# mlelarge/graph_neural_net

Measured on AMD Instinct MI355X. Metric: graph-pairs/sec FGNN fwd+bwd, N=50 regular pairs, higher is better.
Workload: dtype f32

## Files before the change

graph_neural_net_amd/_lib.py:

```python
import ctypes as C
import os

import torch

_HERE = os.path.dirname(os.path.abspath(__file__))
LIB_PATH = os.environ.get('FGNN_LIB') or os.path.join(_HERE, 'libfgnn_hip.so')

FGNN_H = 32
FGNN_TILE = 32
FGNN_MAX_DEPTH = 3
FGNN_RANGE_WG = 256
FGNN_LSAP_MAX_N = 2048
FGNN_QAP_MAX_N = 256
FGNN_QAPW_MAX_N = 256
FGNN_SPECTRAL_MAX_N = 256
FGNN_SPECTRAL_MAX_POWERS = 8
FGNN_SCORE_SPLIT = 4

c_float_p = C.c_void_p


class Slab(C.Structure):
    _fields_ = [('ptr', C.c_void_p), ('gstride', C.c_longlong), ('ldp', C.c_longlong), ('C', C.c_int),
                ('nrm', C.c_void_p), ('beta', C.c_void_p)]
# ... 38 lines not shown
                ('dxb', C.c_void_p), ('dxb_gstride', C.c_longlong), ('dxb_ld', C.c_longlong),
                ('accumulate_dx', C.c_int), ('accumulate_dxb', C.c_int),
                ('wpart', C.c_void_p)]


class Mlp64PackJob(C.Structure):
    _fields_ = [('W', C.c_void_p * 3), ('bias', C.c_void_p * 3), ('cin', C.c_int), ('packed', C.c_void_p)]


class MlpBwdArgs(C.Structure):
    _fields_ = [('G', C.c_int), ('N', C.c_int), ('depth', C.c_int),
                ('nvalid', C.c_void_p),
                ('a', Slab), ('b', Slab),
                ('W', C.c_void_p * FGNN_MAX_DEPTH),
                ('bias', C.c_void_p * FGNN_MAX_DEPTH),
                ('dy', C.c_void_p), ('dgstride', C.c_longlong), ('ldd', C.c_longlong),
                ('z', C.c_void_p), ('zgstride', C.c_longlong), ('ldz', C.c_longlong),
                ('coef', C.c_void_p), ('s12', C.c_void_p), ('znrm', C.c_void_p),
                ('dxa', C.c_void_p), ('dxa_gstride', C.c_longlong), ('dxa_ld', C.c_longlong),
                ('dxb', C.c_void_p), ('dxb_gstride', C.c_longlong), ('dxb_ld', C.c_longlong),
                ('accumulate_a', C.c_int), ('accumulate_b', C.c_int),
                ('wpart', C.c_void_p), ('s12part', C.c_void_p), ('packed', C.c_void_p),
                ('s12tiles', C.c_void_p), ('s12_out', C.c_void_p), ('xbits', C.c_void_p), ('xdeg', C.c_void_p),
                ('ranges', C.c_void_p), ('cu_share', C.c_int)]


class Slab16(C.Structure):
    _fields_ = [('ptr', C.c_void_p), ('gstride', C.c_longlong), ('ldp', C.c_longlong), ('C', C.c_int),
                ('nrm', C.c_void_p), ('beta', C.c_void_p)]


class MlpFwd16Args(C.Structure):
    _fields_ = [('G', C.c_int), ('N', C.c_int), ('ldr', C.c_int), ('depth', C.c_int), ('nmlp', C.c_int),
                ('nvalid', C.c_void_p),
                ('a', Slab16), ('b', Slab16),
                ('z', C.c_void_p * 2), ('ldz', C.c_longlong),
                ('part', C.c_void_p * 2), ('cnt', C.c_void_p), ('packed', C.c_void_p), ('ranges', C.c_void_p)]


class MlpBwd16Args(C.Structure):
    _fields_ = [('G', C.c_int), ('N', C.c_int), ('ldr', C.c_int), ('depth', C.c_int),
                ('nvalid', C.c_void_p),
                ('a', Slab16), ('b', Slab16),
                ('dy', C.c_void_p), ('dgstride', C.c_longlong), ('ldd', C.c_longlong),
                ('z', C.c_void_p), ('zgstride', C.c_longlong), ('ldz', C.c_longlong),
                ('coef', C.c_void_p),
                ('dxa', C.c_void_p), ('dxa_gstride', C.c_longlong), ('dxa_ld', C.c_longlong),
# ... 60 lines not shown
    'fgnn_mlp64_pack_multi': [C.POINTER(Mlp64PackJob), _I, _VP],
    'fgnn_mlp64_fwd': [C.POINTER(Mlp64Args), _VP],
    'fgnn_mlp64_bwd': [C.POINTER(Mlp64Args), _VP],
    'fgnn_conv1x1': [_VP, _LL, _LL, _VP, _VP, _LL, _LL, _VP, _I, _VP, _I, _I, _I, _I, _VP, _LL, _LL, _VP],
    'fgnn_conv1x1_dw_chunks': [_I, _I],
    'fgnn_conv1x1_dw': [_VP, _LL, _LL, _VP, _VP, _LL, _LL, _VP, _I, _I, _I, _I, _VP, _VP],
    'fgnn_chan_matmul_fwd': [C.POINTER(Slab), C.POINTER(Slab), _VP, _I, _I, _VP, _LL, _LL, _VP],
    'fgnn_chan_matmul_fwd_ord': [C.POINTER(Slab), C.POINTER(Slab), _VP, _I, _I, _VP, _LL, _LL, _VP, _I, _VP],
    'fgnn_chan_matmul_fwd_fin_supported': [_I],
    'fgnn_chan_matmul_fwd_fin': [C.POINTER(Slab), C.POINTER(Slab), _VP, _VP, _VP, _VP, _VP, _F, _VP, _I, _I, _VP, _LL, _LL, _VP],
    'fgnn_chan_matmul_fwd_fin_ord': [C.POINTER(Slab), C.POINTER(Slab), _VP, _VP, _VP, _VP, _VP, _F, _VP, _I, _I, _VP, _LL, _LL, _VP, _I, _VP],
    'fgnn_colmax_fwd': [C.POINTER(Slab), _VP, _I, _I, _VP, _VP, _VP],
    'fgnn_colmax_fwd_fin_supported': [_I],
    'fgnn_colmax_fwd_fin': [C.POINTER(Slab), _VP, _VP, _VP, _F, _VP, _I, _I, _VP, _VP, _VP],
    'fgnn_score_ce_fwd': [_VP, _VP, _VP, _I, _I, _I, _VP, _VP, _VP, _VP],
    'fgnn_score_row_blocks': [_I, _I],
    'fgnn_score_ce_fwd_blocks': [_VP, _VP, _VP, _I, _I, _I, _I, _VP, _VP, _VP, _VP],
    'fgnn_score_ce_bwd': [_VP, _VP, _VP, _VP, _VP, _VP, _I, _I, _I, _VP, _VP, _VP],
    'fgnn_inv_node_count': [_VP, _I, _VP, _VP],
    'fgnn_score_bwd': [_VP, _VP, _VP, _VP, _I, _I, _I, _VP, _VP, _VP],
    'fgnn_ce_fwd': [_VP, _VP, _I, _I, _VP, _VP, _VP],
    'fgnn_ce_bwd': [_VP, _VP, _VP, _VP, _I, _I, _VP, _VP],
    'fgnn_colmax_bwd': [_VP, _VP, _VP, _I, _I, _I, _VP, _LL, _LL, C.POINTER(Slab), _VP, _VP],
    'fgnn_gn_bwd_stats': [_VP, _LL, _LL, _VP, _LL, _LL, _VP, _VP, _I, _I, _I, _VP, _VP],
    'fgnn_gn_bwd_coef': [_VP, _VP, _VP, _I, _I, _I, _VP, _VP, _VP, _VP],
    'fgnn_gn_bwd_coef_tiles': [_VP, _VP, _VP, _I, _I, _I, _VP, _VP, _VP],
    'fgnn_grad_finalize': [_VP, _I, _I, _I, _I, _VP],
    'fgnn_gn_bwd_apply': [_VP, _LL, _LL, _VP, _LL, _LL, _VP, _VP, _I, _I, _I, _VP, _LL, _LL, _VP],
    'fgnn_mlp_bwd': [C.POINTER(MlpBwdArgs), _VP],
    'fgnn_mlp_bwd_x3': [C.POINTER(MlpBwdArgs), _VP],
    'fgnn_mlp_bwd_pair': [C.POINTER(MlpBwdArgs), C.POINTER(MlpBwdArgs), _VP],
    'fgnn_mlp_bwd_t16': [C.POINTER(MlpBwdArgs), _VP],
    'fgnn_mlp_bwd_t16_supported': [C.POINTER(MlpBwdArgs)],
    'fgnn_mlp_bwd_pair_t16': [C.POINTER(MlpBwdArgs), C.POINTER(MlpBwdArgs), _VP],
    'fgnn_mlp_bwd_pair_x3': [C.POINTER(MlpBwdArgs), C.POINTER(MlpBwdArgs), _VP],
    'fgnn_block1_struct_supported': [_I, _I, _I],
    'fgnn_block1_struct_table_floats': [_I],
    'fgnn_block1_struct_ws_floats': [_I, _I],
    'fgnn_block1_struct_rows': [_I, _I],
    'fgnn_block1_struct_fwd': [_VP, _VP, _I, _I, _VP, _VP, _VP, _VP, _VP, C.c_float, _VP, _VP, _VP, _LL, _LL, _VP, _VP, _VP, _VP, _VP, _VP, _VP],
    'fgnn_block1_struct_bwd': [_VP, _VP, _I, _I, _VP, _VP, _VP, _VP, _VP, _VP, _VP, _VP, _LL, _LL, _VP, _VP, _VP, _VP, _VP, _VP],
    'fgnn_block1_struct_fwd_pack': [_VP, _VP, _I, _I, _VP, _VP, _VP, _VP, _VP, C.c_float, _VP, _VP, _VP, _LL, _LL, _VP, _VP, _VP, _VP, _VP, _VP, _VP, _I, _VP],
    'fgnn_block1_struct_fwd16_pack': [_VP, _VP, _I, _I, _I, _VP, _VP, _VP, _VP, _VP, C.c_float, _VP, _VP, _VP, _LL, _LL, _VP, _VP, _VP, _VP, _VP, _VP, _VP, _I, _VP],
    'fgnn_block1_struct_fwd16': [_VP, _VP, _I, _I, _I, _VP, _VP, _VP, _VP, _VP, C.c_float, _VP, _VP, _VP, _LL, _LL, _VP, _VP, _VP, _VP, _VP, _VP, _VP],
    'fgnn_block1_struct_bwd16': [_VP, _VP, _I, _I, _I, _VP, _VP, _VP, _VP, _VP, _VP, _VP, _VP, _LL, _LL, _VP, _VP, _VP, _VP, _VP, _VP],
    'fgnn_mlp_bwd_coef_tiles_supported': [_I, _I],
    'fgnn_mlp_param_count': [_I, _I],
    'fgnn_reduce_partials': [_VP, _I, _I, _VP, _VP],
    'fgnn_chan_matmul_bwd': [C.POINTER(Slab), C.POINTER(Slab), _VP, _LL, _LL, _VP, _I, _I, _VP, _VP, _LL, _LL, _VP, _VP, _VP],
    'fgnn_chan_matmul_bwd_ord': [C.POINTER(Slab), C.POINTER(Slab), _VP, _LL, _LL, _VP, _I, _I, _VP, _VP, _LL, _LL, _VP, _VP, _VP, _I, _VP],
    'fgnn_sum_scale': [_VP, _I, _I, _F, _VP, _VP],
    'fgnn_adam_step': [_VP, _VP, _VP, _VP, _I, C.c_double, C.c_double, C.c_double, C.c_double, _I, C.c_double, _VP],
    'fgnn_adam_step_dev': [_VP, _VP, _VP, _VP, _I, _VP, _VP, _VP],
    'fgnn_expand_adjacency': [_VP, _VP, _I, _I, _VP, _VP],
    'fgnn_pack_adjacency': [_VP, _VP, _I, _I, _VP, _VP, _VP],
    'fgnn_pack_adjacency_ld': [_VP, _VP, _I, _I, _I, _VP, _VP, _VP],
# ... 133 lines not shown
```

graph_neural_net_amd/csrc/mlp_bwd_t16.hip:

```cpp
#include "fgnn_t16.h"
#include "fgnn_pack.h"

namespace {

using namespace t16;

constexpr int BWD_WG = 256;
constexpr int NW = 8;

DEVI float4 coef_from_sums(const float4 n, const float2 sv, float nv) {
    const float m = nv * nv;
    float4 k;
    k.x = n.x;
    k.y = n.y;
    k.z = m > 0.f ? -n.y * sv.y * n.w / m : 0.f;
    k.w = m > 0.f ? -n.y * sv.x / m : 0.f;
    return k;
}
DEVI int graph_nv(const rsrc_t &rnv, bool ragged, int g, int N) {
    const int v = __builtin_amdgcn_raw_buffer_load_b32(rnv, g * 4, 0, 0);
    return __builtin_amdgcn_readfirstlane(ragged ? v : N);
}

template <int CB>
struct Layout16 {
    static constexpr int DEPTH = 3;
    static constexpr PkBwd PK = pk_bwd(32, CB, DEPTH);
    static constexpr int OFF_W0A = PK.off_w1a, OFF_W0B = PK.off_w1b, OFF_W1 = PK.off_wh, OFF_WT1 = PK.off_wt, OFF_WT2 = PK.off_wt + 16;
    static constexpr int OFF_WT0A = PK.off_wt0a, OFF_WT0B = PK.off_wt0b;
    static constexpr int BIAS_F = PK.bias_f;
    static constexpr int WEIGHT_F = pk_pad_floats(PK.floats);
    static constexpr int NSLOT = 5;
    static constexpr int CIN = 32 + CB;
    static constexpr int PCOUNT = 32 * CIN + 32 + (DEPTH - 1) * (32 * 32 + 32);
    static constexpr int TILE_OFF = WEIGHT_F;
    static constexpr int REC_OFF = TILE_OFF + NW * NSLOT * TILE_F;
    static constexpr int WGK_OFF = REC_OFF + NW * 256;
    static constexpr int LIVE_OFF = WGK_OFF + FGNN_BWD_COEF_GRAPHS * 128;
    static constexpr int MAIN_F = LIVE_OFF + LIVE_LIST_CAP + NW;
    static constexpr int RED_F = NW * PCOUNT;
    static constexpr int LDS_F = MAIN_F > RED_F ? MAIN_F : RED_F;
};

template <int CB, bool PKD, bool SKIP, bool DXB>
__global__ __launch_bounds__(64 * NW, 2) void mlp_bwd_t16_kernel(const fgnn_mlp_bwd_args A, const int tpg, const int total_tiles) {
    extern __shared__ __attribute__((aligned(16))) float smem[];
    using L = Layout16<CB>;
    constexpr bool NB = CB == 32;
    const int lane = threadIdx.x & 63, wv = __builtin_amdgcn_readfirstlane(threadIdx.x >> 6);
    const int px = lane & 15, q = lane >> 4;
    const int P2 = A.N * A.N, hpg = 2 * tpg;
    const View va = make_view(A.a.ptr, A.a.gstride, A.a.ldp, A.G);
    const View vb = make_view(A.b.ptr, A.b.gstride, A.b.ldp, A.G);
    PackedSrc ps = {};
    if constexpr (PKD) ps = make_packed_src(A.xbits, A.xdeg, A.G, A.N);
    const View vdy = make_view(A.dy, A.dgstride, A.ldd, A.G);
    const View vz = make_view(A.z, A.zgstride, A.ldz, A.G);
    const View vdxa = make_view(A.dxa, A.dxa_gstride, A.dxa_ld, A.G);
    const View vdxb = make_view(A.dxb, A.dxb_gstride, A.dxb_ld, A.G);

    float *wl = smem;
    float *my = smem + L::TILE_OFF + wv * (L::NSLOT * TILE_F);
    float *XA = my, *XB = my + TILE_F, *S0 = my + 2 * TILE_F, *S1 = my + 3 * TILE_F, *S2 = my + 4 * TILE_F;
    const int lane_base = tile_lane_base(px, q);

    f32x4 dW0a[4], dW0b[4], dW1[4], dW2[4];
    float db0[2] = {0.f, 0.f}, db1[2] = {0.f, 0.f}, db2[2] = {0.f, 0.f}, dbx[2] = {0.f, 0.f};
#pragma unroll
    for (int k = 0; k < 4; ++k) dW0a[k] = dW0b[k] = dW1[k] = dW2[k] = zero4();

    const int nwg = gridDim.x;
    const int qq = total_tiles / nwg, rem = total_tiles % nwg;
    int T0 = blockIdx.x * qq + ((int)blockIdx.x < rem ? (int)blockIdx.x : rem);
    int T1 = T0 + qq + ((int)blockIdx.x < rem ? 1 : 0);
    if constexpr (SKIP) {
        T0 = A.ranges[blockIdx.x];
        T1 = A.ranges[blockIdx.x + 1];
    }
    const int H0 = 2 * T0, H1 = 2 * T1;
// ... 75 lines not shown
            }
            rec[lane] = k4;
            if (NB && A.b.nrm) rec[32 + lane] = reinterpret_cast<const float4 *>(A.b.nrm)[(long long)g * A.b.C + lane];
        }
    };
    auto read_records = [&]() {
#pragma unroll
        for (int s = 0; s < 8; ++s) {
            const float4 k4 = rec[chan_s(s) + chan_q(q)];
            kx[s] = k4.x;
            ky[s] = k4.y;
            kz[s] = k4.z;
            kw[s] = k4.w;
            if (NB && A.b.nrm) {
                const float4 n = rec[32 + chan_s(s) + chan_q(q)];
                mean[s] = n.x;
                av[s] = n.y;
            }
        }
    };

    constexpr int NXB = CB == 32 ? 8 : 1;
    float xa[8], xb[NXB], dyr[8], zr[8];
    auto load_x = [&](int h) {
        const bool act = h < H1;
        const int g = __builtin_amdgcn_readfirstlane(act ? h / hpg : 0);
        const int p = (act ? h - g * hpg : 0) * 16 + px;
        const bool inb = act && p < P2;
        load8(xa, va, lane_voff(va, q, p, inb), g * va.gs4);
        if constexpr (CB == 32) {
            load8(xb, vb, lane_voff(vb, q, p, inb), g * vb.gs4);
        } else if constexpr (PKD) {
            int i, jj;
            row_col(p, A.N, rcpN, i, jj);
            const int ob = (inb && q == 0) ? (i * ps.words + (jj >> 5)) * 4 : OOB_OFF;
            const int od = (inb && q == 1 && i == jj) ? i * 4 : OOB_OFF;
            const unsigned w = (unsigned)__builtin_amdgcn_raw_buffer_load_b32(ps.bits, ob, g * ps.N * ps.words * 4, 0);
            const float d = __builtin_bit_cast(float, __builtin_amdgcn_raw_buffer_load_b32(ps.deg, od, g * ps.N * 4, 0));
            xb[0] = q == 0 ? (((w >> (jj & 31)) & 1u) ? 1.f : 0.f) : d;
        } else {
            xb[0] = buf_load(vb, (inb && q < 2) ? q * vb.ld4 + 4 * p : OOB_OFF, g * vb.gs4);
        }
    };
    auto load_dyz = [&](int h) {
        const bool act = h < H1;
        const int g = __builtin_amdgcn_readfirstlane(act ? h / hpg : 0);
        const int p = (act ? h - g * hpg : 0) * 16 + px;
        const bool inb = act && p < P2;
        load8(dyr, vdy, lane_voff(vdy, q, p, inb), g * vdy.gs4);
        load8(zr, vz, lane_voff(vz, q, p, inb), g * vz.gs4);
    };

    int h = next_half(SKIP ? H0 : H0 + wv);
    load_x(h);
    int cached_g = -1, cur_nv = A.N;

    if (from_tiles) {
        const int g1 = T1 > T0 ? (T1 - 1) / tpg : g0 - 1;
        float2 *scr = reinterpret_cast<float2 *>(smem + L::TILE_OFF);
        const int cc = threadIdx.x & 31, sl = threadIdx.x >> 5;
        for (int g = g0; g <= g1; ++g) {
            float p1 = 0.f, p2 = 0.f;
            constexpr int TS = (64 * NW) / 32, U = 8;
            for (int t0 = sl; t0 < tpg; t0 += TS * U) {
                float2 v[U];
#pragma unroll
                for (int k = 0; k < U; ++k) {
                    const int t = t0 + TS * k;
                    v[k] = reinterpret_cast<const float2 *>(A.s12tiles)[((long long)g * tpg + (t < tpg ? t : 0)) * FGNN_H + cc];
                }
#pragma unroll
                for (int k = 0; k < U; ++k) {
// ... 63 lines not shown
            }
            stage8(XA, lane_base, xa);
            if constexpr (CB == 32) {
                stage8(XB, lane_base, yb);
            } else {
                if (q < 2) XB[8 * q * TLD + px] = yb[0];
            }
            f32x4 acc[2];
            load_bias(acc, wl + L::BIAS_F, 0, q);
            gemm32<L::OFF_W0A>(acc, wl, xa, lane);
            if constexpr (CB == 32) gemm32<L::OFF_W0B>(acc, wl, yb, lane);
            else gemm2<L::OFF_W0B>(acc, wl, q < 2 ? yb[0] : 0.f, lane);
            load_x(hn);
#pragma unroll
            for (int s = 0; s < 8; ++s) h1[s] = relu1(acc[s >> 2][s & 3]);
            stage8(S0, lane_base, h1);
            load_bias(acc, wl + L::BIAS_F, 1, q);
            gemm32<L::OFF_W1>(acc, wl, h1, lane);
#pragma unroll
            for (int s = 0; s < 8; ++s) h2[s] = relu1(acc[s >> 2][s & 3]);
            stage8(S1, lane_base, h2);
        }
        float dpre[8];
#pragma unroll
        for (int s = 0; s < 8; ++s) dpre[s] = fmaf(kz[s], zr[s] - kx[s], fmaf(ky[s], dyr[s], kw[s]));
        if (!full) {
#pragma unroll
            for (int s = 0; s < 8; ++s) dpre[s] = valid ? dpre[s] : 0.f;
        }
        stage8(S2, lane_base, dpre);
        load_dyz(hn);
        __builtin_amdgcn_sched_barrier(0);
        {
            f32x4 a2[2];
            a2[0] = a2[1] = zero4();
            gemm32<L::OFF_WT2>(a2, wl, dpre, lane);
            wgrad16(dW2, db2, S2, S1, lane);
#pragma unroll
            for (int s = 0; s < 8; ++s) dpre[s] = h2[s] > 0.f ? a2[s >> 2][s & 3] : 0.f;
        }
        __builtin_amdgcn_sched_barrier(0);
        stage8(S1, lane_base, dpre);
        {
            f32x4 a2[2];
            a2[0] = a2[1] = zero4();
            gemm32<L::OFF_WT1>(a2, wl, dpre, lane);
// ... 76 lines not shown
            red[32 * CIN + 32 + 1024 + c1] = db1[1];
            red[32 * CIN + 32 + 1056 + 1024 + c0] = db2[0];
            red[32 * CIN + 32 + 1056 + 1024 + c1] = db2[1];
        }
    }
    __syncthreads();
    static_assert(PCOUNT % 4 == 0, "partials are summed four at a time");
    float4 *out = reinterpret_cast<float4 *>(A.wpart + (long long)blockIdx.x * PCOUNT);
    const float4 *part4 = reinterpret_cast<const float4 *>(smem);
    for (int e = threadIdx.x; e < PCOUNT / 4; e += 64 * NW) {
        float4 a = part4[e];
#pragma unroll
        for (int w = 1; w < NW; ++w) {
            const float4 b = part4[w * (PCOUNT / 4) + e];
            a.x += b.x;
            a.y += b.y;
            a.z += b.z;
            a.w += b.w;
        }
        out[e] = a;
    }
}

template <int CB, bool PKD, bool SKIP, bool DXB>
int launch16(const fgnn_mlp_bwd_args *a, int tpg, int total, hipStream_t st) {
    constexpr int LDS = Layout16<CB>::LDS_F * 4;
    static_assert(LDS <= 160 * 1024, "LDS budget");
    static LdsAttrCache attr_cache;
    (void)fgnn_raise_lds(attr_cache, (const void *)mlp_bwd_t16_kernel<CB, PKD, SKIP, DXB>, LDS);
    hipLaunchKernelGGL((mlp_bwd_t16_kernel<CB, PKD, SKIP, DXB>), dim3(a->cu_share == 2 && !SKIP ? BWD_WG / 2 : BWD_WG), dim3(64 * NW), LDS, st, *a,
                       tpg, total);
    FGNN_LAUNCH_CHECK();
    return 0;
}
template <int CB, bool PKD, bool DXB>
int launch16s(const fgnn_mlp_bwd_args *a, int tpg, int total, hipStream_t st) {
    return a->ranges ? launch16<CB, PKD, true, DXB>(a, tpg, total, st) : launch16<CB, PKD, false, DXB>(a, tpg, total, st);
}

}

extern "C" int fgnn_mlp_bwd_t16_supported(const fgnn_mlp_bwd_args *a) {
    if (!a || a->depth != 3 || a->a.C != 32 || a->a.nrm || !a->dxa || a->accumulate_a || a->accumulate_b || !a->packed || a->N > 256) return 0;
    if (a->b.C == 32) return (a->b.nrm && a->dxb && !a->xbits) ? 1 : 0;
    if (a->b.C == 2) return (!a->b.nrm && !a->dxb) ? 1 : 0;
    return 0;
}

extern "C" int fgnn_mlp_bwd_t16(const fgnn_mlp_bwd_args *a, void *stream) {
    FGNN_CHECK(a != nullptr, "fgnn_mlp_bwd_t16: null args");
    FGNN_CHECK(fgnn_mlp_bwd_t16_supported(a), "fgnn_mlp_bwd_t16: built for depth 3, slab a = 32 raw channels with dx stored, slab b = 32 normalised "
               "channels with dx stored or 2 raw channels without dx, an operand image of kind 5, N <= 256; use fgnn_mlp_bwd");
    FGNN_CHECK(a->G > 0 && a->N > 0 && a->a.ptr && (a->b.ptr || (a->xbits && a->b.C == 2)), "fgnn_mlp_bwd_t16: bad G / N / slabs");
    FGNN_CHECK(!a->xbits || a->xdeg, "fgnn_mlp_bwd_t16: xbits without xdeg (fgnn_adjacency_degree)");
    FGNN_CHECK(a->dy && a->z && a->wpart, "fgnn_mlp_bwd_t16: missing dy/z/wpart");
    FGNN_CHECK(a->coef || (a->s12 && a->znrm) || (a->s12tiles && a->znrm), "fgnn_mlp_bwd_t16: need coef, or s12 + znrm, or s12tiles + znrm");
    FGNN_CHECK(BWD_WG == fgnn_mlp_bwd_num_workgroups() && BWD_WG == FGNN_RANGE_WG, "fgnn_mlp_bwd_t16: workgroup count differs from fgnn_mlp_bwd");
    {
        const long long lim = 0x7fffffffll / 4, G = a->G;
        FGNN_CHECK(G * a->a.gstride < lim && G * a->b.gstride < lim && G * a->dgstride < lim && G * a->zgstride < lim &&
                   G * a->dxa_gstride < lim && G * a->dxb_gstride < lim,
                   "fgnn_mlp_bwd_t16: a tensor exceeds 2 GiB (32-bit buffer addressing); split the batch");
    }
    for (int l = 0; l < a->depth; ++l) FGNN_CHECK(a->W[l] && a->bias[l], "fgnn_mlp_bwd_t16: missing weights layer %d", l);
    const int tpg = fgnn_tiles_per_graph(a->N);
    const long long total = (long long)a->G * tpg;
    FGNN_CHECK(total < (1ll << 29), "fgnn_mlp_bwd_t16: too many tiles");
    FGNN_CHECK(!a->ranges || (a->nvalid && !a->s12tiles), "fgnn_mlp_bwd_t16: ranges need nvalid and exclude s12tiles");
    FGNN_CHECK(!a->s12tiles || fgnn_mlp_bwd_coef_tiles_supported(a->G, a->N), "fgnn_mlp_bwd_t16: s12tiles needs a workgroup's tile range to span <= %d graphs",
               FGNN_BWD_COEF_GRAPHS);
    hipStream_t st = (hipStream_t)stream;
    if (a->b.C == 32) return launch16s<32, false, true>(a, tpg, (int)total, st);
    if (a->xbits) return launch16s<2, true, false>(a, tpg, (int)total, st);
    return launch16s<2, false, false>(a, tpg, (int)total, st);
}
```

graph_neural_net_amd/csrc/pool_score.hip:

```cpp
#include <float.h>
#include "fgnn_common.h"
#include "fgnn_norm.h"

namespace {

__global__ __launch_bounds__(256) void colmax_fwd_kernel(const fgnn_slab y, const int *nvalid, int G, int N, float *e,
                                                         int *idx) {
    const long long t = (long long)blockIdx.x * (blockDim.x / WAVE) + (threadIdx.x / WAVE);
    const int C = y.C;
    if (t >= (long long)G * C * N) return;
    const int lane = threadIdx.x & 63;
    const int i = (int)(t % N);
    const int gc = (int)(t / N);
    const int g = gc / C, c = gc - g * C;
    const int nv = nvalid_of(nvalid, g, N);
    float best = 0.f;
    int bi = 0;
    if (i < nv) {
        const float *row = y.ptr + (long long)g * y.gstride + (long long)c * y.ldp + (long long)i * N;
        float mean = 0.f, a = 1.f, be = 0.f;
        if (y.nrm) {
            const float4 n = reinterpret_cast<const float4 *>(y.nrm)[gc];
            mean = n.x;
            a = n.y;
// ... 232 lines not shown
        }
    } else {
        for (int p = tid; p < N * N; p += 256) {
            const int i = (int)(((float)p + 0.5f) * invN);
            const int j = p - i * N;
            const int bi = staged ? sidx[i] : idx[(long long)gc * N + i];
            const float d = staged ? sde[i] : (i < nv ? de[(long long)gc * N + i] : 0.f);
            mat[p] = (j == bi) ? d : 0.f;
        }
    }
    if (s12) {
        if (late && tid < nv) {
            s1 += dlate;
            s2 += dlate * (zlate - mean);
        }
        s1 = wave_sum(s1);
        s2 = wave_sum(s2);
        if (lane == 0) {
            red[wave][0] = s1;
            red[wave][1] = s2;
        }
        __syncthreads();
        if (tid < 2) s12[(long long)gc * 2 + tid] = (red[0][tid] + red[1][tid]) + (red[2][tid] + red[3][tid]);
    }
}

DEVI void copy_to_lds256(float *dst, const float *src, int n, int tid) {
    constexpr int U = 8;
    int done = 0;
    if (((reinterpret_cast<unsigned long long>(src) | reinterpret_cast<unsigned long long>(dst)) & 15ull) == 0) {
        const int n4 = n >> 2;
        const float4 *s4 = reinterpret_cast<const float4 *>(src);
        float4 *d4 = reinterpret_cast<float4 *>(dst);
        for (int e0 = tid; e0 < n4; e0 += 256 * U) {
            float4 v[U];
#pragma unroll
            for (int k = 0; k < U; ++k) {
                const int e = e0 + 256 * k;
                v[k] = s4[e < n4 ? e : 0];
            }
#pragma unroll
            for (int k = 0; k < U; ++k) {
                const int e = e0 + 256 * k;
                if (e < n4) d4[e] = v[k];
            }
        }
// ... 293 lines not shown
                                   const int *nvalid, int G, int N, float *e, int *idx, void *stream) {
    FGNN_CHECK(y && y->ptr && y->nrm && part && cnt && e && idx && G > 0 && N > 0 && y->C > 0, "fgnn_colmax_fwd_fin: bad arguments");
    FGNN_CHECK(N <= 64, "fgnn_colmax_fwd_fin: N=%d > 64 (use fgnn_gn_finalize + fgnn_colmax_fwd)", N);
    const ColmaxFin F = {part, cnt, gn_weight, eps, fgnn_tiles_per_graph(N)};
    hipLaunchKernelGGL(colmax_fwd_lds_kernel<true>, dim3((unsigned)((G * y->C + 3) / 4)), dim3(256), 0, (hipStream_t)stream, *y,
                       nvalid, G, N, e, idx, F);
    FGNN_LAUNCH_CHECK();
    return 0;
}

extern "C" int fgnn_colmax_bwd(const float *de, const int *idx, const int *nvalid, int G, int C, int N, float *dy,
                               long long gstride, long long ldp, const fgnn_slab *y, float *s12, void *stream) {
    FGNN_CHECK(de && idx && dy && G > 0 && C > 0 && N > 0, "fgnn_colmax_bwd: bad arguments");
    FGNN_CHECK(!s12 || (y && y->ptr && y->nrm && y->C == C), "fgnn_colmax_bwd: s12 needs the normalised input slab");
    fgnn_slab ys = {};
    if (s12) ys = *y;
    const int tot = G * C;
    hipLaunchKernelGGL(colmax_bwd_kernel, dim3((unsigned)tot), dim3(256), 0, (hipStream_t)stream, de,
                       idx, nvalid, G, C, N, dy, gstride, ldp, ys, s12);
    FGNN_LAUNCH_CHECK();
    return 0;
}

static int score_lds_bytes(int C, int N) { return (2 * C * N + 4) * (int)sizeof(float); }
static int score_bwd_lds_bytes(int C, int N, bool stage, int csplit = CSPLIT) {
    const int cper = (C + csplit - 1) / csplit;
    return (2 * cper * N + (stage ? N * (N + 1) : 0)) * (int)sizeof(float);
}
template <bool CE>
static int launch_score_bwd(const float *e1, const float *e2, const float *scores, const float *lse,
                            const float *dscores, const int *nvalid, const float *gscale, int B, int C, int N,
                            float *de1, float *de2, hipStream_t st) {
    const bool stage = score_bwd_lds_bytes(C, N, true) <= 160 * 1024 && (N <= 64 || (long long)B * CSPLIT >= 256);
    const int csplit = (long long)B * CSPLIT < 256 ? CSPLIT_SMALL : CSPLIT;
    const int lds = score_bwd_lds_bytes(C, N, stage, stage ? csplit : CSPLIT);
    FGNN_CHECK(lds <= 160 * 1024, "score backward: C*N=%d too large for LDS staging", C * N);
    if (stage) {
        if (lds > 64 * 1024)
            (void)hipFuncSetAttribute((const void *)score_bwd_kernel<CE, true>, hipFuncAttributeMaxDynamicSharedMemorySize, lds);
        hipLaunchKernelGGL((score_bwd_kernel<CE, true>), dim3(B, csplit), dim3(256), lds, st, e1, e2, scores, lse, dscores,
                           nvalid, gscale, C, N, de1, de2);
    } else {
        const int cper = (C + CSPLIT - 1) / CSPLIT;
        const int SB_BLK = (long long)B * CSPLIT * ((N + 63) / 64) >= 512 ? 64 : 16;
        const int big = (N + 1) * SB_BLK > N * (SB_BLK + 1) ? (N + 1) * SB_BLK : N * (SB_BLK + 1);
        const int lds2 = (2 * cper * N + big) * (int)sizeof(float);
// ... 64 lines not shown
```

graph_neural_net_amd/engine.py:

```python
import ctypes as C
import os

import torch

from . import _lib
from .engine_base import EngineBase

EPS = 1e-05


class ParamLayout:

    def __init__(self, original_features_num=2, num_blocks=4, in_features=32, out_features=32, depth_of_mlp=3):
        if in_features != _lib.FGNN_H or out_features != _lib.FGNN_H:
            raise RuntimeError('the fused engine is built for in_features = out_features = 32 (got %d, %d); other widths '
                               'run through the per-layer modules (layers.MlpBlock_Real)' % (in_features, out_features))
        if not 1 <= depth_of_mlp <= _lib.FGNN_MAX_DEPTH:
            raise RuntimeError('depth_of_mlp must be in 1..%d' % _lib.FGNN_MAX_DEPTH)
        if original_features_num not in (2, 32):
            raise RuntimeError('the fused engine is built for original_features_num = 2 or 32 (got %d); other widths run '
                               'through the per-layer modules (layers.MlpBlock_Real)' % original_features_num)
        self.c0 = original_features_num
        self.num_blocks = num_blocks
        self.depth = depth_of_mlp
# ... 92 lines not shown

    def keys(self):
        return list(self._items)

    def clear(self):
        self._items.clear()

    def __len__(self):
        return len(self._items)

    def __iter__(self):
        return iter(list(self._items))

    def values(self):
        return [e for e, _ in self._items.values()]


class FgnnEngine(EngineBase):
    SKIP_PADDING_TILES = True
    MM_ORDER = True
    PAIR_BWD = os.environ.get('FGNN_PAIR_BWD', '1') != '0'
    PACK_IN_STRUCT = os.environ.get('FGNN_PACK_IN_STRUCT', '1') != '0'
    T16 = os.environ.get('FGNN_T16', 'pair,bwd')

    MFMA = os.environ.get('FGNN_MFMA', 'f32')

    BLOCK1 = os.environ.get('FGNN_BLOCK1', 'generic')
    GN_FINALIZE = ('fgnn_gn_finalize', 'fgnn_gn_finalize2')

    def __init__(self, layout, G, N, device, ragged=False, cu_share=0, mfma=None, block1=None):
        _lib.load()
        self.T16 = type(self).T16
        self.cu_share = int(cu_share)
        mfma = self.MFMA if mfma is None else mfma
        if mfma not in ('f32', 'x3'):
            raise ValueError("mfma must be 'f32' or 'x3' (got %r)" % (mfma,))
        self.x3 = (mfma == 'x3' and not ragged and layout.depth == 3 and layout.c0 in (2, 32))
        block1 = self.BLOCK1 if block1 is None else block1
        if block1 not in ('generic', 'structured'):
            raise ValueError("block1 must be 'generic' or 'structured' (got %r)" % (block1,))
        self.struct1 = (block1 == 'structured' and cu_share == 0
                        and bool(_lib.load().fgnn_block1_struct_supported(N, layout.depth, layout.c0)))
        super().__init__(layout, G, N, device, ragged)
        self.P = N * N
        self.ldp = _round_up(self.P, 32)
        self.tpg = _lib.tiles_per_graph(N)
        self._gn_args = (EPS,)
        K = layout.num_blocks
        f32 = dict(dtype=torch.float32, device=device)
        self._act = act = lambda: torch.empty(G * 32 * self.ldp, **f32)
        self.z = {(k, j): act() for k in range(1, K + 1) for j in (1, 2, 3)}
        self.mult = {k: act() for k in range(1, K + 1)}
        self.part = [torch.empty(G * self.tpg * 32 * 2, **f32) for _ in range(2)]
        self.cnt = torch.empty(G * 2 * self.tpg, **f32)
        self.mm_order = (torch.empty(G, dtype=torch.int32, device=device)
# ... 165 lines not shown
        (w1, _), (w2, _) = self._w3(params, 1), self._w3(params, 2)
        r1, r2 = self.layout.mlp[(1, 1)], self.layout.mlp[(1, 2)]
        _lib.call('fgnn_block1_struct_bwd', _lib.ptr(self.xbits), self._nv(), self.G, self.N, _lib.ptr(S['tab']), w1, w2,
                  _lib.ptr(self.nrm[(1, 1)]), _lib.ptr(self.nrm[(1, 2)]),
                  C.c_void_p(self._w(params, r1['gn_b'])), C.c_void_p(self._w(params, r2['gn_b'])),
                  _lib.ptr(W['dmult']), 32 * self.ldp, self.ldp, _lib.ptr(S['ws']),
                  _lib.ptr(W['wpart'][(1, 1)]), _lib.ptr(W['wpart'][(1, 2)]), _lib.ptr(W['s12'][(1, 1)]), _lib.ptr(W['s12'][(1, 2)]),
                  _lib.stream_ptr())

    def _partial_rows(self):
        nwg = super()._partial_rows()
        if self.cu_share == 2 and self.ranges is None:
            nwg //= 2
        return nwg

    def _coef(self, kj, slot):
        W = self._bwd
        _lib.call('fgnn_gn_bwd_coef', _lib.ptr(W['s12'][kj]), _lib.ptr(self.nrm[kj]), self._nv(), self.G, 32, self.N,
                  _lib.ptr(W['coef'][slot]), None, None, _lib.stream_ptr())

    def _mlp_bwd(self, params, k, j, a, b, dy, coef, dxa, dxb, acc_a, acc_b, emit=False, dx_strides=None):
        args = self._mlp_bwd_args(params, k, j, a, b, dy, coef, dxa, dxb, acc_a, acc_b, emit, dx_strides)
        entry = 'fgnn_mlp_bwd_x3' if (self.x3 and j != 3) else 'fgnn_mlp_bwd'
        if j == 3 and b is not None and self._t16_bwd3(b.C) and _lib.load().fgnn_mlp_bwd_t16_supported(C.byref(args)):
            entry = 'fgnn_mlp_bwd_t16'
        elif self._packs[('b', k, j)][0] == 5:
            args.packed = None
        _lib.call(entry, C.byref(args), _lib.stream_ptr(),
                  tag='mlp_bwd[cin=%d,dx=%d]' % (a.C + (b.C if b is not None else 0),
                                                (a.C if dxa is not None else 0) + (b.C if (b is not None and dxb is not None) else 0)))

    def _mlp_bwd_pair(self, params, k, sin, din, emit):
        W = self._bwd
        a1 = self._mlp_bwd_args(params, k, 1, sin, None, W['dy1'], None, None, None, False, False, False, None)
        a2 = self._mlp_bwd_args(params, k, 2, sin, None, W['dy2'], None, din, None, True, False, emit, None)
        entry = 'fgnn_mlp_bwd_pair_x3' if self.x3 else ('fgnn_mlp_bwd_pair_t16' if self._t16_pair(sin.C) else 'fgnn_mlp_bwd_pair')
        _lib.call(entry, C.byref(a1), C.byref(a2), _lib.stream_ptr(),
                  tag='mlp_bwd_pair[cin=%d,dx=%d]' % (sin.C, sin.C if din is not None else 0))

    def _mlp_bwd_args(self, params, k, j, a, b, dy, coef, dxa, dxb, acc_a, acc_b, emit, dx_strides):
        L = self.layout
        W = self._bwd
        rec = L.mlp[(k, j)]
        gs = 32 * self.ldp
        args = _lib.MlpBwdArgs()
        args.G, args.N, args.depth = self.G, self.N, L.depth
        args.nvalid = self.nvalid.data_ptr() if self.nvalid is not None else None
        args.a = a
        if b is not None:
            args.b = b
        for l in range(L.depth):
            args.W[l] = self._w(params, rec['w'][l])
            args.bias[l] = self._w(params, rec['b'][l])
        args.dy, args.dgstride, args.ldd = dy.data_ptr(), gs, self.ldp
        args.z, args.zgstride, args.ldz = self.z[(k, j)].data_ptr(), gs, self.ldp
        if isinstance(coef, str):
            args.s12tiles = W['s12part'].data_ptr()
            args.s12_out = W['s12'][(k, j)].data_ptr()
            args.znrm = self.nrm[(k, j)].data_ptr()
        elif coef is not None:
            args.coef = coef.data_ptr()
        else:
            args.s12 = W['s12'][(k, j)].data_ptr()
            args.znrm = self.nrm[(k, j)].data_ptr()
        dgs, dld = (gs, self.ldp) if dx_strides is None else dx_strides
        if dxa is not None:
            args.dxa, args.dxa_gstride, args.dxa_ld = dxa.data_ptr(), (gs if (b is not None and dx_strides is not None) else dgs), \
                (self.ldp if (b is not None and dx_strides is not None) else dld)
        if dxb is not None:
            args.dxb, args.dxb_gstride, args.dxb_ld = dxb.data_ptr(), dgs, dld
        args.accumulate_a, args.accumulate_b = int(acc_a), int(acc_b)
        args.wpart = W['wpart'][(k, j)].data_ptr()
        args.packed = self._packs[('b', k, j)][4].data_ptr()
        self._packed_input(args, k)
        if self.ranges is not None:
            args.ranges = self.ranges.data_ptr()
        args.cu_share = self.cu_share
        if emit:
            args.s12part = W['s12part'].data_ptr()
        return args

    def backward_from_dE(self, params, grads, dE, finalize=True, dx=None):
        L = self.layout
        W = self._alloc_bwd()
        st = _lib.stream_ptr()
        gs = 32 * self.ldp
        K = L.num_blocks
        in_prologue = bool(_lib.load().fgnn_mlp_bwd_coef_tiles_supported(self.G, self.N)) and self.ranges is None
        dy = W['dy'][0]
        out = self._slab_z(K, 3, params)
        _lib.call('fgnn_colmax_bwd', _lib.ptr(dE), _lib.ptr(self.idx), self._nv(), self.G, 32, self.N,
                  _lib.ptr(dy), gs, self.ldp, C.byref(out), _lib.ptr(W['s12'][(K, 3)]), st)
        for k in range(K, 0, -1):
            sin = self._slab_in(k, params)
            first = (k == 1)
            din = None if first else W['dy'][(K - k + 1) % 2]
            dxs = None
            if first and dx is not None:
                if self.xbits is not None or self.x3 or tuple(dx.shape) != (self.G, L.c0, self.N, self.N) or dx.dtype != torch.float32 \
                        or not dx.is_contiguous():
                    raise RuntimeError('FgnnEngine: the input gradient needs a dense fp32 input, the fp32-MFMA kernels (mfma="f32") '
                                       'and a contiguous (G, c0, N, N) fp32 dx')
                din, dxs = dx, (L.c0 * self.P, self.P)
            self._mlp_bwd(params, k, 3, self._slab_raw(self.mult[k]), sin, dy,
                          None if k == K else ('tiles' if in_prologue else W['coef'][2]), W['dmult'], din, False, False, dx_strides=dxs)
            if first and self.struct1 and self.xbits is not None and dxs is None:
                self._struct_bwd(params)
                dy = din
                continue
            ya, yb = self._slab_z(k, 1, params), self._slab_z(k, 2, params)
            _lib.call('fgnn_chan_matmul_bwd_ord', C.byref(ya), C.byref(yb), _lib.ptr(W['dmult']), gs, self.ldp,
                      self._nv(), self.G, self.N, _lib.ptr(W['dy1']), _lib.ptr(W['dy2']), gs, self.ldp,
                      _lib.ptr(W['s12'][(k, 1)]), _lib.ptr(W['s12'][(k, 2)]),
                      _lib.ptr(self.mm_order) if self.mm_order is not None else None, self._fill(), st, tag='fgnn_chan_matmul_bwd')
            if first:
# ... 56 lines not shown
```

include/fgnn_hip.h:

```cpp
#ifndef FGNN_HIP_H
#define FGNN_HIP_H

#ifdef __cplusplus
extern "C" {
#endif

#define FGNN_H 32
#define FGNN_TILE 32
#define FGNN_MAX_DEPTH 3

typedef struct {
    const float *ptr;
    long long gstride;
    long long ldp;
    int C;
    const float *nrm;
    const float *beta;
} fgnn_slab;

const char *fgnn_last_error(void);
int fgnn_version(void);
int fgnn_tiles_per_graph(int N);
int fgnn_mlp_bwd_num_workgroups(void);

// ... 141 lines not shown
                    int *idx , void *stream);
int fgnn_colmax_fwd_fin_supported(int N);
int fgnn_colmax_fwd_fin(const fgnn_slab *y, const float *part, const float *cnt, const float *gn_weight, float eps,
                        const int *nvalid, int G, int N, float *e, int *idx, void *stream);

#define FGNN_SCORE_SPLIT 4
int fgnn_score_ce_fwd(const float *e1, const float *e2, const int *nvalid, int B, int C, int N,
                      float *scores, float *lse, float *pair_loss, void *stream);
int fgnn_score_row_blocks(int B, int N);
int fgnn_score_ce_fwd_blocks(const float *e1, const float *e2, const int *nvalid, int B, int C, int N, int row_blocks,
                             float *scores, float *lse, float *pair_loss, void *stream);
int fgnn_score_ce_bwd(const float *e1, const float *e2, const float *scores, const float *lse,
                      const int *nvalid, const float *gscale, int B, int C, int N,
                      float *de1, float *de2, void *stream);

int fgnn_ce_fwd(const float *scores, const int *nvalid, int B, int N, float *lse, float *pair_loss, void *stream);
int fgnn_ce_bwd(const float *scores, const float *lse, const int *nvalid, const float *gscale, int B, int N,
                float *dscores, void *stream);
int fgnn_score_bwd(const float *e1, const float *e2, const float *dscores, const int *nvalid,
                   int B, int C, int N, float *de1, float *de2, void *stream);

int fgnn_colmax_bwd(const float *de, const int *idx, const int *nvalid, int G, int C, int N,
                    float *dy, long long gstride, long long ldp, const fgnn_slab *y, float *s12, void *stream);

int fgnn_gn_bwd_stats(const float *dy, long long dgstride, long long ldd,
                      const float *z, long long zgstride, long long ldz, const float *nrm,
                      const int *nvalid, int G, int C, int N, float *s12 , void *stream);
int fgnn_gn_bwd_coef(const float *s12, const float *nrm, const int *nvalid, int G, int C, int N,
                     float *coef , float *dgn_w , float *dgn_b ,
                     void *stream);
int fgnn_gn_bwd_coef_tiles(const float *s12part, const float *nrm, const int *nvalid, int G, int C, int N,
                           float *s12, float *coef, void *stream);
int fgnn_gn_bwd_apply(const float *dy, long long dgstride, long long ldd,
                      const float *z, long long zgstride, long long ldz, const float *coef,
                      const int *nvalid, int G, int C, int N, float *dz, long long ogstride, long long ldo, void *stream);

typedef struct {
    int G, N, depth;
    const int *nvalid;
    fgnn_slab a, b;
    const float *W[FGNN_MAX_DEPTH];
    const float *bias[FGNN_MAX_DEPTH];
    const float *dy;  long long dgstride, ldd;
    const float *z;   long long zgstride, ldz;
    const float *coef;
    const float *s12;
    const float *znrm;
    float *dxa; long long dxa_gstride, dxa_ld;
    float *dxb; long long dxb_gstride, dxb_ld;
    int accumulate_a, accumulate_b;
    float *wpart;
    float *s12part;
    const float *packed;
    const float *s12tiles;
    float *s12_out;
    const unsigned *xbits;
    const float *xdeg;
    const int *ranges;
    int cu_share;
} fgnn_mlp_bwd_args;
int fgnn_mlp_bwd(const fgnn_mlp_bwd_args *args, void *stream);
int fgnn_mlp_bwd_x3(const fgnn_mlp_bwd_args *args, void *stream);
int fgnn_mlp_bwd_pair(const fgnn_mlp_bwd_args *m1, const fgnn_mlp_bwd_args *m2, void *stream);
int fgnn_mlp_bwd_pair_x3(const fgnn_mlp_bwd_args *m1, const fgnn_mlp_bwd_args *m2, void *stream);
int fgnn_mlp_bwd_t16_supported(const fgnn_mlp_bwd_args *args);
int fgnn_mlp_bwd_t16(const fgnn_mlp_bwd_args *args, void *stream);
int fgnn_mlp_bwd_pair_t16(const fgnn_mlp_bwd_args *m1, const fgnn_mlp_bwd_args *m2, void *stream);
#define FGNN_BWD_COEF_GRAPHS 4
int fgnn_mlp_bwd_coef_tiles_supported(int G, int N);
int fgnn_mlp_param_count(int Cin, int depth);
int fgnn_reduce_partials(const float *wpart, int num_wg, int count, float *out, void *stream);

#define FGNN_MAX_GRAD_JOBS 16
typedef struct {
    const float *wpart; int count; float *out;
    const float *s12; const float *nrm; float *dgn_w; float *dgn_b;
    int rows;
    float scale;
    const float *scale_dev;
} fgnn_grad_job;
int fgnn_grad_finalize(const fgnn_grad_job *jobs, int njobs, int num_wg, int G, int C, void *stream);
int fgnn_inv_node_count(const int *nvalid, int B, float *out, void *stream);

int fgnn_chan_matmul_bwd(const fgnn_slab *ya, const fgnn_slab *yb, const float *dm, long long dmgstride, long long ldm,
                         const int *nvalid, int G, int N,
                         float *da, float *db, long long ogstride, long long ldo,
                         float *s12a ,
                         float *s12b , void *stream);
int fgnn_chan_matmul_bwd_ord(const fgnn_slab *ya, const fgnn_slab *yb, const float *dm, long long dmgstride, long long ldm,
// ... 193 lines not shown
```

Before: 42510.

## Fuse colmax backward scatter into t16 MLP backward via virtual dy

Replaces the colmax backward pass, which scattered dE into a dense dy slab, with a stats-only kernel that computes only the group-norm s12 sums. The last block's t16 MLP backward kernel then rebuilds dy on the fly from dE and the argmax indices, masking entries whose index does not match the column. This removes writing and re-reading the full N×N×C dy tensor. In exchange the kernel does extra per-element index loads and compares, and the path only covers fixed-size batches with 32-channel slabs.

```diff
diff --git a/graph_neural_net_amd/_lib.py b/graph_neural_net_amd/_lib.py
--- a/graph_neural_net_amd/_lib.py
+++ b/graph_neural_net_amd/_lib.py
@@ -84,7 +84,8 @@
                 ('accumulate_a', C.c_int), ('accumulate_b', C.c_int),
                 ('wpart', C.c_void_p), ('s12part', C.c_void_p), ('packed', C.c_void_p),
                 ('s12tiles', C.c_void_p), ('s12_out', C.c_void_p), ('xbits', C.c_void_p), ('xdeg', C.c_void_p),
-                ('ranges', C.c_void_p), ('cu_share', C.c_int)]
+                ('ranges', C.c_void_p), ('cu_share', C.c_int),
+                ('dE', C.c_void_p), ('idx', C.c_void_p)]
 
 
 class Slab16(C.Structure):
@@ -191,6 +192,7 @@
     'fgnn_ce_fwd': [_VP, _VP, _I, _I, _VP, _VP, _VP],
     'fgnn_ce_bwd': [_VP, _VP, _VP, _VP, _I, _I, _VP, _VP],
     'fgnn_colmax_bwd': [_VP, _VP, _VP, _I, _I, _I, _VP, _LL, _LL, C.POINTER(Slab), _VP, _VP],
+    'fgnn_colmax_bwd_stats': [_VP, _VP, _I, _I, _I, C.POINTER(Slab), _VP, _VP],
     'fgnn_gn_bwd_stats': [_VP, _LL, _LL, _VP, _LL, _LL, _VP, _VP, _I, _I, _I, _VP, _VP],
     'fgnn_gn_bwd_coef': [_VP, _VP, _VP, _I, _I, _I, _VP, _VP, _VP, _VP],
     'fgnn_gn_bwd_coef_tiles': [_VP, _VP, _VP, _I, _I, _I, _VP, _VP, _VP],
@@ -201,6 +203,7 @@
     'fgnn_mlp_bwd_pair': [C.POINTER(MlpBwdArgs), C.POINTER(MlpBwdArgs), _VP],
     'fgnn_mlp_bwd_t16': [C.POINTER(MlpBwdArgs), _VP],
     'fgnn_mlp_bwd_t16_supported': [C.POINTER(MlpBwdArgs)],
+    'fgnn_mlp_bwd_t16_vdy_supported': [C.POINTER(MlpBwdArgs)],
     'fgnn_mlp_bwd_pair_t16': [C.POINTER(MlpBwdArgs), C.POINTER(MlpBwdArgs), _VP],
     'fgnn_mlp_bwd_pair_x3': [C.POINTER(MlpBwdArgs), C.POINTER(MlpBwdArgs), _VP],
     'fgnn_block1_struct_supported': [_I, _I, _I],
diff --git a/graph_neural_net_amd/csrc/mlp_bwd_t16.hip b/graph_neural_net_amd/csrc/mlp_bwd_t16.hip
--- a/graph_neural_net_amd/csrc/mlp_bwd_t16.hip
+++ b/graph_neural_net_amd/csrc/mlp_bwd_t16.hip
@@ -42,7 +42,7 @@
     static constexpr int LDS_F = MAIN_F > RED_F ? MAIN_F : RED_F;
 };
 
-template <int CB, bool PKD, bool SKIP, bool DXB>
+template <int CB, bool PKD, bool SKIP, bool DXB, bool VDY>
 __global__ __launch_bounds__(64 * NW, 2) void mlp_bwd_t16_kernel(const fgnn_mlp_bwd_args A, const int tpg, const int total_tiles) {
     extern __shared__ __attribute__((aligned(16))) float smem[];
     using L = Layout16<CB>;
@@ -54,7 +54,9 @@
     const View vb = make_view(A.b.ptr, A.b.gstride, A.b.ldp, A.G);
     PackedSrc ps = {};
     if constexpr (PKD) ps = make_packed_src(A.xbits, A.xdeg, A.G, A.N);
-    const View vdy = make_view(A.dy, A.dgstride, A.ldd, A.G);
+    const View vdy = make_view(VDY ? nullptr : A.dy, A.dgstride, A.ldd, VDY ? 0 : A.G);
+    const rsrc_t rde = __builtin_amdgcn_make_buffer_rsrc(const_cast<float *>(VDY ? A.dE : nullptr), 0, VDY ? A.G * 32 * A.N * 4 : 0, 0x00020000);
+    const rsrc_t rix = __builtin_amdgcn_make_buffer_rsrc(const_cast<int *>(VDY ? A.idx : nullptr), 0, VDY ? A.G * 32 * A.N * 4 : 0, 0x00020000);
     const View vz = make_view(A.z, A.zgstride, A.ldz, A.G);
     const View vdxa = make_view(A.dxa, A.dxa_gstride, A.dxa_ld, A.G);
     const View vdxb = make_view(A.dxb, A.dxb_gstride, A.dxb_ld, A.G);
@@ -176,6 +178,7 @@
 
     constexpr int NXB = CB == 32 ? 8 : 1;
     float xa[8], xb[NXB], dyr[8], zr[8];
+    int dix[VDY ? 8 : 1], dcol = 0;
     auto load_x = [&](int h) {
         const bool act = h < H1;
         const int g = __builtin_amdgcn_readfirstlane(act ? h / hpg : 0);
@@ -201,7 +204,17 @@
         const int g = __builtin_amdgcn_readfirstlane(act ? h / hpg : 0);
         const int p = (act ? h - g * hpg : 0) * 16 + px;
         const bool inb = act && p < P2;
-        load8(dyr, vdy, lane_voff(vdy, q, p, inb), g * vdy.gs4);
+        if constexpr (VDY) {
+            int i;
+            row_col(p, A.N, rcpN, i, dcol);
+            const int voff = inb ? (chan_q(q) * A.N + i) * 4 : OOB_OFF, s0 = g * 32 * A.N * 4;
+#pragma unroll
+            for (int s = 0; s < 8; ++s) dyr[s] = __builtin_bit_cast(float, __builtin_amdgcn_raw_buffer_load_b32(rde, voff, s0 + chan_s(s) * A.N * 4, 0));
+#pragma unroll
+            for (int s = 0; s < 8; ++s) dix[s] = __builtin_amdgcn_raw_buffer_load_b32(rix, voff, s0 + chan_s(s) * A.N * 4, 0);
+        } else {
+            load8(dyr, vdy, lane_voff(vdy, q, p, inb), g * vdy.gs4);
+        }
         load8(zr, vz, lane_voff(vz, q, p, inb), g * vz.gs4);
     };
 
@@ -311,6 +324,10 @@
             stage8(S1, lane_base, h2);
         }
         float dpre[8];
+        if constexpr (VDY) {
+#pragma unroll
+            for (int s = 0; s < 8; ++s) dyr[s] = dix[s] == dcol ? dyr[s] : 0.f;
+        }
 #pragma unroll
         for (int s = 0; s < 8; ++s) dpre[s] = fmaf(kz[s], zr[s] - kx[s], fmaf(ky[s], dyr[s], kw[s]));
         if (!full) {
@@ -433,13 +450,13 @@
     }
 }
 
-template <int CB, bool PKD, bool SKIP, bool DXB>
+template <int CB, bool PKD, bool SKIP, bool DXB, bool VDY = false>
 int launch16(const fgnn_mlp_bwd_args *a, int tpg, int total, hipStream_t st) {
     constexpr int LDS = Layout16<CB>::LDS_F * 4;
     static_assert(LDS <= 160 * 1024, "LDS budget");
     static LdsAttrCache attr_cache;
-    (void)fgnn_raise_lds(attr_cache, (const void *)mlp_bwd_t16_kernel<CB, PKD, SKIP, DXB>, LDS);
-    hipLaunchKernelGGL((mlp_bwd_t16_kernel<CB, PKD, SKIP, DXB>), dim3(a->cu_share == 2 && !SKIP ? BWD_WG / 2 : BWD_WG), dim3(64 * NW), LDS, st, *a,
+    (void)fgnn_raise_lds(attr_cache, (const void *)mlp_bwd_t16_kernel<CB, PKD, SKIP, DXB, VDY>, LDS);
+    hipLaunchKernelGGL((mlp_bwd_t16_kernel<CB, PKD, SKIP, DXB, VDY>), dim3(a->cu_share == 2 && !SKIP ? BWD_WG / 2 : BWD_WG), dim3(64 * NW), LDS, st, *a,
                        tpg, total);
     FGNN_LAUNCH_CHECK();
     return 0;
@@ -456,6 +473,10 @@
     if (a->b.C == 32) return (a->b.nrm && a->dxb && !a->xbits) ? 1 : 0;
     if (a->b.C == 2) return (!a->b.nrm && !a->dxb) ? 1 : 0;
     return 0;
+}
+
+extern "C" int fgnn_mlp_bwd_t16_vdy_supported(const fgnn_mlp_bwd_args *a) {
+    return (fgnn_mlp_bwd_t16_supported(a) && a->b.C == 32 && !a->nvalid && !a->ranges) ? 1 : 0;
 }
 
 extern "C" int fgnn_mlp_bwd_t16(const fgnn_mlp_bwd_args *a, void *stream) {
@@ -464,7 +485,10 @@
                "channels with dx stored or 2 raw channels without dx, an operand image of kind 5, N <= 256; use fgnn_mlp_bwd");
     FGNN_CHECK(a->G > 0 && a->N > 0 && a->a.ptr && (a->b.ptr || (a->xbits && a->b.C == 2)), "fgnn_mlp_bwd_t16: bad G / N / slabs");
     FGNN_CHECK(!a->xbits || a->xdeg, "fgnn_mlp_bwd_t16: xbits without xdeg (fgnn_adjacency_degree)");
-    FGNN_CHECK(a->dy && a->z && a->wpart, "fgnn_mlp_bwd_t16: missing dy/z/wpart");
+    const bool vdy = a->dE || a->idx;
+    FGNN_CHECK(!vdy || (a->dE && a->idx && !a->dy && fgnn_mlp_bwd_t16_vdy_supported(a)),
+               "fgnn_mlp_bwd_t16: dE / idx come together, replace dy and need slab b = 32 channels and a constant-size batch");
+    FGNN_CHECK((a->dy || vdy) && a->z && a->wpart, "fgnn_mlp_bwd_t16: missing dy/z/wpart");
     FGNN_CHECK(a->coef || (a->s12 && a->znrm) || (a->s12tiles && a->znrm), "fgnn_mlp_bwd_t16: need coef, or s12 + znrm, or s12tiles + znrm");
     FGNN_CHECK(BWD_WG == fgnn_mlp_bwd_num_workgroups() && BWD_WG == FGNN_RANGE_WG, "fgnn_mlp_bwd_t16: workgroup count differs from fgnn_mlp_bwd");
     {
@@ -481,6 +505,7 @@
     FGNN_CHECK(!a->s12tiles || fgnn_mlp_bwd_coef_tiles_supported(a->G, a->N), "fgnn_mlp_bwd_t16: s12tiles needs a workgroup's tile range to span <= %d graphs",
                FGNN_BWD_COEF_GRAPHS);
     hipStream_t st = (hipStream_t)stream;
+    if (vdy) return launch16<32, false, false, true, true>(a, tpg, (int)total, st);
     if (a->b.C == 32) return launch16s<32, false, true>(a, tpg, (int)total, st);
     if (a->xbits) return launch16s<2, true, false>(a, tpg, (int)total, st);
     return launch16s<2, false, false>(a, tpg, (int)total, st);
diff --git a/graph_neural_net_amd/csrc/pool_score.hip b/graph_neural_net_amd/csrc/pool_score.hip
--- a/graph_neural_net_amd/csrc/pool_score.hip
+++ b/graph_neural_net_amd/csrc/pool_score.hip
@@ -278,6 +278,48 @@
         }
         __syncthreads();
         if (tid < 2) s12[(long long)gc * 2 + tid] = (red[0][tid] + red[1][tid]) + (red[2][tid] + red[3][tid]);
+    }
+}
+
+constexpr int CMS_WAVES = 4;
+__global__ __launch_bounds__(64 * CMS_WAVES) void colmax_bwd_stats_kernel(const float *de, const int *idx, int GC, int N,
+                                                                          const fgnn_slab y, float *s12) {
+    const int lane = threadIdx.x & 63;
+    const int gc = blockIdx.x * CMS_WAVES + (threadIdx.x >> 6);
+    if (gc >= GC) return;
+    const int g = gc / y.C, c = gc - g * y.C;
+    const float *zm = y.ptr + (long long)g * y.gstride + (long long)c * y.ldp;
+    const float mean = y.nrm[(long long)gc * 4];
+    int bi[4];
+    float d[4], zv[4];
+#pragma unroll
+    for (int w = 0; w < 4; ++w) {
+        const int i = 64 * w + lane;
+        const long long t = (long long)gc * N + (i < N ? i : 0);
+        bi[w] = idx[t];
+        d[w] = de[t];
+    }
+#pragma unroll
+    for (int w = 0; w < 4; ++w) {
+        const int i = 64 * w + lane;
+        int b = bi[w];
+        b = b < 0 ? 0 : (b < N ? b : N - 1);
+        zv[w] = zm[(long long)(i < N ? i : 0) * N + b];
+    }
+    float r1[4], r2[4];
+#pragma unroll
+    for (int w = 0; w < 4; ++w) {
+        float s1 = 0.f, s2 = 0.f;
+        if (64 * w + lane < N) {
+            s1 += d[w];
+            s2 += d[w] * (zv[w] - mean);
+        }
+        r1[w] = 64 * w < N ? wave_sum(s1) : 0.f;
+        r2[w] = 64 * w < N ? wave_sum(s2) : 0.f;
+    }
+    if (lane == 0) {
+        s12[(long long)gc * 2] = (r1[0] + r1[1]) + (r1[2] + r1[3]);
+        s12[(long long)gc * 2 + 1] = (r2[0] + r2[1]) + (r2[2] + r2[3]);
     }
 }
 
@@ -617,6 +659,17 @@
     return 0;
 }
 
+extern "C" int fgnn_colmax_bwd_stats(const float *de, const int *idx, int G, int C, int N, const fgnn_slab *y, float *s12, void *stream) {
+    FGNN_CHECK(de && idx && s12 && G > 0 && C > 0 && N > 0, "fgnn_colmax_bwd_stats: bad arguments");
+    FGNN_CHECK(N <= 256, "fgnn_colmax_bwd_stats: N=%d > 256; use fgnn_colmax_bwd", N);
+    FGNN_CHECK(y && y->ptr && y->nrm && y->C == C, "fgnn_colmax_bwd_stats: needs the normalised input slab");
+    const int tot = G * C;
+    hipLaunchKernelGGL(colmax_bwd_stats_kernel, dim3((unsigned)((tot + CMS_WAVES - 1) / CMS_WAVES)), dim3(64 * CMS_WAVES), 0,
+                       (hipStream_t)stream, de, idx, tot, N, *y, s12);
+    FGNN_LAUNCH_CHECK();
+    return 0;
+}
+
 static int score_lds_bytes(int C, int N) { return (2 * C * N + 4) * (int)sizeof(float); }
 static int score_bwd_lds_bytes(int C, int N, bool stage, int csplit = CSPLIT) {
     const int cper = (C + csplit - 1) / csplit;
diff --git a/graph_neural_net_amd/engine.py b/graph_neural_net_amd/engine.py
--- a/graph_neural_net_amd/engine.py
+++ b/graph_neural_net_amd/engine.py
@@ -138,6 +138,7 @@
     PAIR_BWD = os.environ.get('FGNN_PAIR_BWD', '1') != '0'
     PACK_IN_STRUCT = os.environ.get('FGNN_PACK_IN_STRUCT', '1') != '0'
     T16 = os.environ.get('FGNN_T16', 'pair,bwd')
+    VDY = os.environ.get('FGNN_VDY', '1') != '0'
 
     MFMA = os.environ.get('FGNN_MFMA', 'f32')
 
@@ -147,6 +148,8 @@
     def __init__(self, layout, G, N, device, ragged=False, cu_share=0, mfma=None, block1=None):
         _lib.load()
         self.T16 = type(self).T16
+        self.VDY = type(self).VDY
+        self._vdy_built = None
         self.cu_share = int(cu_share)
         mfma = self.MFMA if mfma is None else mfma
         if mfma not in ('f32', 'x3'):
@@ -358,7 +361,9 @@
     def _mlp_bwd(self, params, k, j, a, b, dy, coef, dxa, dxb, acc_a, acc_b, emit=False, dx_strides=None):
         args = self._mlp_bwd_args(params, k, j, a, b, dy, coef, dxa, dxb, acc_a, acc_b, emit, dx_strides)
         entry = 'fgnn_mlp_bwd_x3' if (self.x3 and j != 3) else 'fgnn_mlp_bwd'
-        if j == 3 and b is not None and self._t16_bwd3(b.C) and _lib.load().fgnn_mlp_bwd_t16_supported(C.byref(args)):
+        if isinstance(dy, tuple):
+            entry = 'fgnn_mlp_bwd_t16'
+        elif j == 3 and b is not None and self._t16_bwd3(b.C) and _lib.load().fgnn_mlp_bwd_t16_supported(C.byref(args)):
             entry = 'fgnn_mlp_bwd_t16'
         elif self._packs[('b', k, j)][0] == 5:
             args.packed = None
@@ -388,7 +393,11 @@
         for l in range(L.depth):
             args.W[l] = self._w(params, rec['w'][l])
             args.bias[l] = self._w(params, rec['b'][l])
-        args.dy, args.dgstride, args.ldd = dy.data_ptr(), gs, self.ldp
+        if isinstance(dy, tuple):
+            args.dE, args.idx = dy[0].data_ptr(), dy[1].data_ptr()
+            args.dgstride, args.ldd = gs, self.ldp
+        else:
+            args.dy, args.dgstride, args.ldd = dy.data_ptr(), gs, self.ldp
         args.z, args.zgstride, args.ldz = self.z[(k, j)].data_ptr(), gs, self.ldp
         if isinstance(coef, str):
             args.s12tiles = W['s12part'].data_ptr()
@@ -416,6 +425,17 @@
             args.s12part = W['s12part'].data_ptr()
         return args
 
+    def _vdy(self, params, dx):
+        K = self.layout.num_blocks
+        if not (self.VDY and K > 1 and dx is None and self.nvalid is None and self.ranges is None and self._t16_bwd3(32)):
+            return False
+        if self._vdy_built is None:
+            W = self._bwd
+            args = self._mlp_bwd_args(params, K, 3, self._slab_raw(self.mult[K]), self._slab_in(K, params), W['dy'][0], None,
+                                      W['dmult'], W['dy'][1], False, False, False, None)
+            self._vdy_built = bool(_lib.load().fgnn_mlp_bwd_t16_vdy_supported(C.byref(args)))
+        return self._vdy_built
+
     def backward_from_dE(self, params, grads, dE, finalize=True, dx=None):
         L = self.layout
         W = self._alloc_bwd()
@@ -425,8 +445,13 @@
         in_prologue = bool(_lib.load().fgnn_mlp_bwd_coef_tiles_supported(self.G, self.N)) and self.ranges is None
         dy = W['dy'][0]
         out = self._slab_z(K, 3, params)
-        _lib.call('fgnn_colmax_bwd', _lib.ptr(dE), _lib.ptr(self.idx), self._nv(), self.G, 32, self.N,
-                  _lib.ptr(dy), gs, self.ldp, C.byref(out), _lib.ptr(W['s12'][(K, 3)]), st)
+        if self._vdy(params, dx):
+            _lib.call('fgnn_colmax_bwd_stats', _lib.ptr(dE), _lib.ptr(self.idx), self.G, 32, self.N, C.byref(out),
+                      _lib.ptr(W['s12'][(K, 3)]), st)
+            dy = (dE, self.idx)
+        else:
+            _lib.call('fgnn_colmax_bwd', _lib.ptr(dE), _lib.ptr(self.idx), self._nv(), self.G, 32, self.N,
+                      _lib.ptr(dy), gs, self.ldp, C.byref(out), _lib.ptr(W['s12'][(K, 3)]), st)
         for k in range(K, 0, -1):
             sin = self._slab_in(k, params)
             first = (k == 1)
diff --git a/include/fgnn_hip.h b/include/fgnn_hip.h
--- a/include/fgnn_hip.h
+++ b/include/fgnn_hip.h
@@ -187,6 +187,7 @@
 
 int fgnn_colmax_bwd(const float *de, const int *idx, const int *nvalid, int G, int C, int N,
                     float *dy, long long gstride, long long ldp, const fgnn_slab *y, float *s12, void *stream);
+int fgnn_colmax_bwd_stats(const float *de, const int *idx, int G, int C, int N, const fgnn_slab *y, float *s12, void *stream);
 
 int fgnn_gn_bwd_stats(const float *dy, long long dgstride, long long ldd,
                       const float *z, long long zgstride, long long ldz, const float *nrm,
@@ -223,6 +224,8 @@
     const float *xdeg;
     const int *ranges;
     int cu_share;
+    const float *dE;
+    const int *idx;
 } fgnn_mlp_bwd_args;
 int fgnn_mlp_bwd(const fgnn_mlp_bwd_args *args, void *stream);
 int fgnn_mlp_bwd_x3(const fgnn_mlp_bwd_args *args, void *stream);
@@ -230,6 +233,7 @@
 int fgnn_mlp_bwd_pair_x3(const fgnn_mlp_bwd_args *m1, const fgnn_mlp_bwd_args *m2, void *stream);
 int fgnn_mlp_bwd_t16_supported(const fgnn_mlp_bwd_args *args);
 int fgnn_mlp_bwd_t16(const fgnn_mlp_bwd_args *args, void *stream);
+int fgnn_mlp_bwd_t16_vdy_supported(const fgnn_mlp_bwd_args *args);
 int fgnn_mlp_bwd_pair_t16(const fgnn_mlp_bwd_args *m1, const fgnn_mlp_bwd_args *m2, void *stream);
 #define FGNN_BWD_COEF_GRAPHS 4
 int fgnn_mlp_bwd_coef_tiles_supported(int G, int N);
```

Result: no change. 42820 (median of 6 runs) (+0.7%).
